# simone7monaco/NO-NODE-comparison

Measured on AMD Instinct MI355X. Metric: N-body trajectories/s (B×T, N=20 rollout) + pos-MSE vs ref, 1/2/4/8 MI355X, higher is better.
Workload: dtype fp32 (fp16x3 split-MFMA, fp32 accumulate, f32 guard); 1 GPU; C2: EGNO forward (4 layers, hidden 64, 2 modes), charged N=20, T=10, B=512 per GPU; batch_per_gpu=512, global_batch=512, n_balls=20, layer_workgroups=256, edges=fixed, parallelism=batch-sharded replicas x1 (no collective)

## Files before the change

### no-node-comparison_amd/csrc/nonode.hip

```cpp
#include "nonode_common.h"

namespace nonode_tu {
thread_local std::string g_err;
}

namespace {

struct ProfState {
  std::mutex mu;
  bool on = false;
  int cap = 0, n = 0;
  hipEvent_t* ev = nullptr;
  int* kind = nullptr;
} g_prof;

constexpr int PROF_SIM_CHARGED = 4, PROF_SIM_GRAVITY = 5, PROF_EDGE_BWD0 = 6, PROF_EDGE_BWD1 = 7;

struct ProfScope {
  int slot = -1;
  hipStream_t s;
  ProfScope(int kind, hipStream_t stream) : s(stream) {
    if (!g_prof.on) return;
    std::lock_guard<std::mutex> lk(g_prof.mu);
    if (g_prof.n >= g_prof.cap) return;
// ... 147 lines not shown
#else
#define STAMP_DECL
#define STAMP(i) do {} while (0)
#define STAMP_FLUSH
#endif

enum { EGNO = 0, SEGNO = 1 };

struct LayerArgs {
  const float* __restrict__ h; const float* __restrict__ x; const float* __restrict__ v;
  const float* __restrict__ ef; const float* __restrict__ blob;
  float* h_out; float* x_out; float* v_out;
  float* pp_h[2]; float* pp_x[2]; float* pp_v[2];
  int steps;
  int fuse, keep;
  float* m_out; float* f_out;
  float* sv_h; float* sv_x; float* sv_v;
  long long sv_n;
  int n_total, n_graphs, N, ne, ef_mod, recurrent;
  int cg, cpg, n_units, ct, s_rows;
  float inv_deg, dt, cw;
  int use_perm;
  unsigned short chunk_of[256];
};

size_t layer_lds_floats(int ct, int s_rows, int keep = 0) {
  return 8192 + EDGE_STAGE_FLOATS + (size_t)ct * 16 * ROWP * 3 + (size_t)s_rows * (ROWP + 4) +
         (size_t)ct * 16 * 4 * 2 + (keep ? (size_t)ct * 16 * (ROWP + 4) : 0);
}

#ifndef NONODE_NODE_PAIR
#define NONODE_NODE_PAIR 1
#endif
template <int VARIANT, int KF, int NW, bool OPT, bool SAVE = false>
__device__ __forceinline__ void egnn_layer_body(const LayerArgs& p, int (*s_cut)[NW + 1]) {
  constexpr bool PAIR = NW == 4;
  constexpr bool TRIPLE = PAIR && VARIANT == EGNO;
  [[maybe_unused]] constexpr bool stamp_here = VARIANT == EGNO && NW == 4 && !OPT;
  constexpr bool rnorm = OPT && VARIANT == EGNO;
  constexpr bool ctanh = OPT && VARIANT == SEGNO;
  extern __shared__ __attribute__((aligned(16))) float smem[];
  const int tid = threadIdx.x, lane = tid & 63, wave = tid >> 6, e = lane & 15, g = lane >> 4;
  const int N = p.N, Nm1 = N - 1;
  float* sW = smem;
  float* sV = sW + 8192;
  float* sP = sV + EDGE_STAGE_FLOATS;
  float* sQ = sP + p.ct * 16 * ROWP;
  float* sX = sQ + p.s_rows * ROWP;
  float* sM = sX + p.s_rows * 4;
  float* sF = sM + 2 * p.ct * 16 * ROWP;
  const int slotM = p.ct * 16 * ROWP, slotF = p.ct * 16 * 4;
  float* sH = sF + 2 * slotF;
  float* sVl = sH + p.ct * 16 * ROWP;
  const bool fused = VARIANT == SEGNO && p.fuse != 0, keep = fused && p.keep != 0;

  for (int i = tid; i < 2048; i += NW * 64) reinterpret_cast<f4*>(sW)[i] = reinterpret_cast<const f4*>(p.blob + OFF_H16)[i];
  if (tid < EDGE_STAGE_FLOATS / 4)
    reinterpret_cast<f4*>(sV)[tid] = reinterpret_cast<const f4*>(p.blob + OFF_FEAT)[tid];
  const float bc2 = p.blob[OFF_SCAL + 0];
  const float bv2 = p.blob[OFF_SCAL + 1];
  const unsigned us_w2 = h16_us(p.blob + OFF_SCAL, HS_W2), us_wc1 = h16_us(p.blob + OFF_SCAL, HS_WC1);
  const float* vFEAT_ = sV;
  const float* vB2_ = sV + 512 + V_B2 * 64;
  const float* vBC1_ = sV + 512 + V_BC1 * 64;
  const float* vWC2_ = sV + 512 + V_WC2 * 64;

  const int G = gridDim.x;
  const int cb = p.use_perm ? (int)p.chunk_of[blockIdx.x] : (int)blockIdx.x;
  const int ch0 = (int)(((long long)cb * p.n_units) / G) * p.cpg;
  const int ch1 = (int)(((long long)(cb + 1) * p.n_units) / G) * p.cpg;
  __syncthreads();
  for (int i = tid; i < 2 * p.ct * 16 * ROWP; i += NW * 64) sM[i] = 0.f;
  for (int i = tid; i < 2 * p.ct * 16 * 4; i += NW * 64) sF[i] = 0.f;
  auto chunk_at = [&](int ci, int& rbase, int& nend, int& s0, int& S) __attribute__((always_inline)) {
    if (p.cpg == 1) {
      const int g_lo = ci * p.cg, g_hi = min(g_lo + p.cg, p.n_graphs);
      rbase = g_lo * N; nend = g_hi * N; s0 = rbase; S = nend - rbase;
    } else {
      const int gi = ci / p.cpg, part = ci - gi * p.cpg;
      s0 = gi * N; S = N;
      rbase = s0 + part * 16 * p.ct; nend = min(rbase + 16 * p.ct, s0 + N);
    }
  };
  auto proj_jobs = [&](int rbase, int nend, int S) __attribute__((always_inline)) {
    const int ctc = (nend - rbase + 15) >> 4;
    return p.cpg == 1 ? ctc : ctc + ((S + 15) >> 4);
  };
  auto proj_tile = [&](const f4 (&hin)[4], const float* blob, int local, bool valid) __attribute__((always_inline)) {
    f4 ap[4], aq[4];
    load_vp(ap, blob + OFF_VEC + V_B1 * 64, g);
#pragma unroll
    for (int mt = 0; mt < 4; ++mt) aq[mt] = f4{0.f, 0.f, 0.f, 0.f};
    if (__builtin_expect(__any(amax_ecl(hin) > H16_LIMIT), 0)) {
      mfma_dense<4>(ap, blob + OFF_WA, hin, lane);
      mfma_dense<4>(aq, blob + OFF_WB, hin, lane);
    } else {
      h8 xh[2], xl[2];
      h16_split(hin, xh, xl);
      mfma_h16(ap, reinterpret_cast<const h8*>(blob + OFF_H16N + H_WA * 4096), xh, xl, lane, h16_us(blob + OFF_SCAL, HS_N + H_WA));
      mfma_h16(aq, reinterpret_cast<const h8*>(blob + OFF_H16N + H_WB * 4096), xh, xl, lane, h16_us(blob + OFF_SCAL, HS_N + H_WB));
    }
    float sa = 0.f;
#pragma unroll
    for (int mt = 0; mt < 4; ++mt)
#pragma unroll
      for (int q = 0; q < 4; ++q) sa += fabsf(ap[mt][q]) + fabsf(aq[mt][q]);
    sa = group_sum(sa);
    if (valid) {
      store_ecl(sP + local * ROWP, ap, g);
      store_ecl(sQ + local * ROWP, aq, g);
      if (g == 0) sX[local * 4 + 3] = __builtin_isfinite(sa) ? 1.f : 0.f;
    }
  };
  auto proj_job = [&](const float* __restrict__ hI, const float* blob, int rbase, int nend, int s0, int S,
                      int job) __attribute__((always_inline)) {
    int joff = 0;
    asm volatile("" : "+s"(joff));
    blob += joff;
    if (p.cpg == 1) {
      const int local = job * 16 + e;
      const bool valid = rbase + local < nend;
      f4 hin[4];
      load_ecl(hin, hI + (size_t)(valid ? rbase + local : nend - 1) * HID, g);
      if (keep && valid) store_ecl(sH + local * ROWP, hin, g);
      proj_tile(hin, blob, local, valid);
      return;
    }
    const int ctc = (nend - rbase + 15) >> 4;
    const bool isP = job < ctc;
    const int local = (isP ? job : job - ctc) * 16 + e;
    int node = isP ? rbase + local : s0 + local;
    const bool valid = isP ? (node < nend) : (local < S);
    node = valid ? node : (isP ? nend - 1 : s0);
    f4 hin[4];
    load_ecl(hin, hI + (size_t)node * HID, g);
    f4 acc[4];
    if (isP) {
      load_vp(acc, blob + OFF_VEC + V_B1 * 64, g);
    } else {
#pragma unroll
      for (int mt = 0; mt < 4; ++mt) acc[mt] = f4{0.f, 0.f, 0.f, 0.f};
    }
    mm64(acc, reinterpret_cast<const h8*>(blob + OFF_H16N + (isP ? H_WA : H_WB) * 4096),
         blob + (isP ? OFF_WA : OFF_WB), hin, lane, h16_us(blob + OFF_SCAL, HS_N + (isP ? H_WA : H_WB)));
    float sa = 0.f;
#pragma unroll
    for (int mt = 0; mt < 4; ++mt)
#pragma unroll
// ... 23 lines not shown
    load_vp(ap0, blob + OFF_VEC + V_B1 * 64, g);
    load_vp(ap1, blob + OFF_VEC + V_B1 * 64, g);
#pragma unroll
    for (int mt = 0; mt < 4; ++mt) aq0[mt] = aq1[mt] = f4{0.f, 0.f, 0.f, 0.f};
    h8 ah[2], al[2], bh[2], bl[2];
    h16_split(h0, ah, al);
    h16_split(h1, bh, bl);
    mfma_h16x2(ap0, ap1, reinterpret_cast<const h8*>(blob + OFF_H16N + H_WA * 4096), ah, al, bh, bl, lane,
               h16_us(blob + OFF_SCAL, HS_N + H_WA));
    mfma_h16x2(aq0, aq1, reinterpret_cast<const h8*>(blob + OFF_H16N + H_WB * 4096), ah, al, bh, bl, lane,
               h16_us(blob + OFF_SCAL, HS_N + H_WB));
    float sa0 = 0.f, sa1 = 0.f;
#pragma unroll
    for (int mt = 0; mt < 4; ++mt)
#pragma unroll
      for (int q = 0; q < 4; ++q) {
        sa0 += fabsf(ap0[mt][q]) + fabsf(aq0[mt][q]);
        sa1 += fabsf(ap1[mt][q]) + fabsf(aq1[mt][q]);
      }
    sa0 = group_sum(sa0);
    sa1 = group_sum(sa1);
    if (v0) {
      store_ecl(sP + l0 * ROWP, ap0, g);
      store_ecl(sQ + l0 * ROWP, aq0, g);
      if (g == 0) sX[l0 * 4 + 3] = __builtin_isfinite(sa0) ? 1.f : 0.f;
    }
    if (v1) {
      store_ecl(sP + l1 * ROWP, ap1, g);
      store_ecl(sQ + l1 * ROWP, aq1, g);
      if (g == 0) sX[l1 * 4 + 3] = __builtin_isfinite(sa1) ? 1.f : 0.f;
    }
  };
  auto load_sx = [&](const float* __restrict__ xI, const float* __restrict__ vI, int s0, int S) __attribute__((always_inline)) {
    for (int i = tid; i < S * 3; i += NW * 64) {
      const int s = i / 3, d = i - 3 * s;
      sX[s * 4 + d] = xI[(size_t)(s0 + s) * 3 + d];
      if (keep) sVl[s * 4 + d] = vI[(size_t)(s0 + s) * 3 + d];
    }
  };
  STAMP_DECL
  int* cut = s_cut[wave];
  int cut_ctc = -1, cut_vl = -1;
  #pragma unroll 1
  for (int step = 0; step < p.steps; ++step) {
  constexpr bool save = VARIANT == SEGNO && SAVE;
  const bool last = step == p.steps - 1;
  const float* __restrict__ hI = step == 0 ? p.h : (save ? p.sv_h + step * p.sv_n * HID : p.pp_h[(step - 1) & 1]);
  const float* __restrict__ xI = step == 0 ? p.x : (save ? p.sv_x + step * p.sv_n * 3 : p.pp_x[(step - 1) & 1]);
  const float* __restrict__ vI = step == 0 ? p.v : (save ? p.sv_v + step * p.sv_n * 3 : p.pp_v[(step - 1) & 1]);
  float* hO = save ? p.sv_h + (step + 1) * p.sv_n * HID : (last ? p.h_out : p.pp_h[step & 1]);
  float* xO = save ? p.sv_x + (step + 1) * p.sv_n * 3 : (last ? p.x_out : p.pp_x[step & 1]);
  float* vO = save ? p.sv_v + (step + 1) * p.sv_n * 3 : (last ? p.v_out : p.pp_v[step & 1]);
  float* mO = p.m_out ? p.m_out + (save ? step * p.sv_n * HID : 0) : nullptr;
  if (!fused || step == 0) {
    int rbase, nend, s0, S;
    chunk_at(ch0, rbase, nend, s0, S);
    load_sx(xI, vI, s0, S);
    const int J = proj_jobs(rbase, nend, S);
    if (NONODE_NODE_PAIR && NW == 4 && VARIANT == EGNO && p.cpg == 1) {
      #pragma unroll 1
      for (int job = 2 * wave; job < J; job += 2 * NW) {
        if (job + 1 < J) proj_job2(hI, p.blob, rbase, nend, job);
        else proj_job(hI, p.blob, rbase, nend, s0, S, job);
      }
    } else {
      #pragma unroll 1
      for (int job = wave; job < J; job += NW) proj_job(hI, p.blob, rbase, nend, s0, S, job);
    }
    STAMP(6);
    __syncthreads();
    STAMP(7);
  }
  #pragma unroll 1
  for (int ci = ch0; ci < ch1; ++ci) {
    int boff = 0;
    asm volatile("" : "+s"(boff));
    const float* blob = p.blob + boff;
    int rbase, nend, s0, S;
    chunk_at(ci, rbase, nend, s0, S);
    const int ctc = (nend - rbase + 15) >> 4;

    {
      const int Vl = (nend - rbase) - 16 * (ctc - 1);
      const int Pk = (Vl <= 4 && Nm1 >= 8) ? 4 : ((Vl <= 8 && Nm1 >= 4) ? 2 : 1);
      const int Kp = Nm1 / Pk;
      const int Ul = Pk == 1 ? Nm1 : Kp + (Nm1 - Pk * Kp);
      const int U = (ctc - 1) * Nm1 + Ul;
      if (ctc != cut_ctc || Vl != cut_vl) {
        cut_ctc = ctc;
        cut_vl = Vl;
        if constexpr (PAIR) {
          unit_split<NW>(ctc, Nm1, Ul, Pk == 1 ? Nm1 : Kp, cut);
        } else {
          const int NWB = min(NW, 3 * ctc);
          for (int i = 0; i <= NW; ++i) cut[i] = i < NWB ? (i * U) / NWB : U;
        }
      }
      const int u1 = cut[wave + 1];
      int u = cut[wave];
      f4 rB2[4], rBC1[4], rWC2[4];
      if (PAIR) {
        load_vp(rB2, vB2_, g);
        load_vp(rBC1, vBC1_, g);
        load_vp(rWC2, vWC2_, g);
      }
      #pragma unroll 1
      while (u < u1) {
        const int tau = min(u / Nm1, ctc - 1);
        const int k_lo = u - tau * Nm1 + 1;
        const int k_hi = min(tau == ctc - 1 ? Ul : Nm1, k_lo + (u1 - u) - 1);
        u += k_hi - k_lo + 1;
        const int P = tau == ctc - 1 ? Pk : 1;
        const int Kq = P == 1 ? Nm1 : Kp;
        const int hp = P == 1 ? 0 : (P == 2 ? e >> 3 : e >> 2);
        const int ee = P == 1 ? e : (P == 2 ? e & 7 : e & 3);
        const int kof = hp * Kq;
        const int kreg = (P - 1) * Kq;
        const int rl = 16 * tau + ee;
        auto lane_k = [&](int k) __attribute__((always_inline)) { return k <= Kq ? k + kof : k + kreg; };
        auto lane_on = [&](int k) __attribute__((always_inline)) { return k <= Kq || hp == 0; };
        const int r = rbase + rl;
        const bool rvalid = r < nend;
        const int rc = rvalid ? r : nend - 1;
        const int gr = rc / N;
        const int n = rc - gr * N;
        const int sb = gr * N - s0;
        const size_t ebase = ((size_t)(gr % p.ef_mod) * N + n) * Nm1;
        int voff = 0;
        asm volatile("" : "+v"(voff));
        const float* vFEAT = vFEAT_ + voff;
        const float* Prow = sP + rl * ROWP;
        const float xr0 = sX[(sb + n) * 4 + 0], xr1 = sX[(sb + n) * 4 + 1], xr2 = sX[(sb + n) * 4 + 2];
        const float xr3 = sX[(sb + n) * 4 + 3];
        f4 msum[4];
#pragma unroll
        for (int mt = 0; mt < 4; ++mt) msum[mt] = f4{0.f, 0.f, 0.f, 0.f};
        float fs0 = 0.f, fs1 = 0.f, fs2 = 0.f;

        const float* ef_seg = p.ef + ebase * p.ne;
        int ef_lane[KF];
#pragma unroll
        for (int kf = 0; kf < KF; ++kf) ef_lane[kf] = n * p.ne + min(max(4 * kf + g - 1, 0), p.ne - 1);
        const int ne_wrap = N * p.ne;
        auto fetch_ef = [&](int k, float (&ev)[KF]) __attribute__((always_inline)) {
          const int sub = (n + k >= N) ? ne_wrap : p.ne;
          const int kne = k * p.ne;
#pragma unroll
          for (int kf = 0; kf < KF; ++kf)
            ev[kf] = ef_seg[ef_lane[kf] + kne - sub];
        };
        auto head = [&](int k, const float (&ev)[KF], f4 (&a)[4], float& r0, float& r1, float& r2)
            __attribute__((always_inline)) {
          int j = n + k;
          j = (j >= N) ? j - N : j;
          const int sl = sb + j;
          const float* xs = sX + sl * 4;
          r0 = xr0 - xs[0]; r1 = xr1 - xs[1]; r2 = xr2 - xs[2];
          float d2 = fmaf(r0, r0, fmaf(r1, r1, r2 * r2));
          if constexpr (rnorm) d2 = radial_norm(d2);
          f4 q4[4];
// ... 242 lines not shown
#pragma unroll
              for (int mo = 0; mo < 4; ++mo) a[mo] = mfma(wf[mo], bv, a[mo]);
            }
          };
          auto coord1 = [&](f4 (&c1)[4], const float* wc2, float r0, float r1, float r2, float& f0, float& f1,
                            float& f2, float& c) __attribute__((always_inline)) {
            silu_ecl(c1);
            c = dot_vp(c1, wc2, g) + bc2;
            float ct = c;
            if constexpr (ctanh) ct = tanhf(c);
            f0 = r0 * ct; f1 = r1 * ct; f2 = r2 * ct;
            if (VARIANT == SEGNO) {
              f0 = fminf(fmaxf(f0, -100.f), 100.f);
              f1 = fminf(fmaxf(f1, -100.f), 100.f);
              f2 = fminf(fmaxf(f2, -100.f), 100.f);
            }
          };
          auto unit1 = [&](int k, int k_end, float (&e0)[KF], auto masked) __attribute__((always_inline)) {
            float en[KF];
            fetch_ef(lane_k(min(k + 1, k_end)), en);
            int loff = 0;
            asm volatile("" : "+v"(loff));
            const h8* w2l = w2h + loff;
            const h8* wc1l = wc1h + loff;
            f4 a[4], m[4];
            float r0, r1, r2, f0, f1, f2, c;
            bool ok;
            head1(lane_k(k), e0, a, r0, r1, r2, ok);
            silu_ecl(a);
            load_vp(m, vB2_ + loff, g);
            {
              h8 ah[2], al[2];
              h16_split(a, ah, al);
              mfma_h16(m, w2l, ah, al, lane, us_w2);
            }
            silu_ecl(m);
            load_vp(a, vBC1_ + loff, g);
            {
              h8 mh[2], ml[2];
              h16_split(m, mh, ml);
              mfma_h16(a, wc1l, mh, ml, lane, us_wc1);
            }
            coord1(a, vWC2_ + loff, r0, r1, r2, f0, f1, f2, c);
            if (__builtin_expect(__any(ok && !__builtin_isfinite(c)), 0)) {
              int kg = k;
              asm volatile("" : "+v"(kg));
              head1(lane_k(kg), e0, a, r0, r1, r2, ok);
              silu_ecl(a);
              load_vp(m, vB2_, g);
              mm64_scaled(m, w2h, a, lane, us_w2);
              silu_ecl(m);
              load_vp(a, vBC1_, g);
              mm64_scaled(a, wc1h, m, lane, us_wc1);
              coord1(a, vWC2_, r0, r1, r2, f0, f1, f2, c);
            }
            if constexpr (decltype(masked)::value) {
              const bool on = lane_on(k);
#pragma unroll
              for (int mt = 0; mt < 4; ++mt)
#pragma unroll
                for (int q = 0; q < 4; ++q) msum[mt][q] = on ? msum[mt][q] + m[mt][q] : msum[mt][q];
              fs0 = on ? fs0 + f0 : fs0; fs1 = on ? fs1 + f1 : fs1; fs2 = on ? fs2 + f2 : fs2;
            } else {
#pragma unroll
              for (int mt = 0; mt < 4; ++mt) msum[mt] += m[mt];
              fs0 += f0; fs1 += f1; fs2 += f2;
            }
#pragma unroll
            for (int kf = 0; kf < KF; ++kf) e0[kf] = en[kf];
          };
          float e0[KF];
          fetch_ef(lane_k(min(k, k_hi)), e0);
          const int ko_hi = min(k_hi, Kq);
#pragma unroll 1
          for (; k <= ko_hi; ++k) unit1(k, ko_hi, e0, std::false_type{});
          if (k <= k_hi) fetch_ef(lane_k(k), e0);
#pragma unroll 1
          for (; k <= k_hi; ++k) unit1(k, k_hi, e0, std::true_type{});
        }
        float e0[KF];
        fetch_ef(lane_k(min(k, k_hi)), e0);
        STAMP(8);
#pragma unroll 1
        for (; k <= k_hi; ++k) {
          float en[KF];
          fetch_ef(lane_k(min(k + 1, k_hi)), en);
          const bool on = lane_on(k);
          int loff = 0;
          asm volatile("" : "+v"(loff));
          const h8* w2l = w2h + loff;
          const h8* wc1l = wc1h + loff;
          const float* vB2l = vB2_ + loff;
          const float* vBC1l = vBC1_ + loff;
          f4 a[4], m[4];
          float r0, r1, r2;
          head(lane_k(k), e0, a, r0, r1, r2);
#pragma unroll
          for (int kf = 0; kf < KF; ++kf) e0[kf] = en[kf];
          STAMP(0);
          silu_ecl(a);
          if (PAIR) {
#pragma unroll
            for (int mt = 0; mt < 4; ++mt) m[mt] = rB2[mt];
          } else {
            load_vp(m, vB2l, g);
          }
          if (__builtin_expect(__any(amax_ecl(a) > H16_LIMIT), 0)) {
            mm64_scaled(m, w2l, a, lane, us_w2);
          } else {
            h8 ah[2], al[2];
            h16_split(a, ah, al);
            mfma_h16(m, w2l, ah, al, lane, us_w2);
          }
          STAMP(1);
          silu_ecl(m);
#pragma unroll
          for (int mt = 0; mt < 4; ++mt)
#pragma unroll
            for (int q = 0; q < 4; ++q) msum[mt][q] = on ? msum[mt][q] + m[mt][q] : msum[mt][q];
          if (PAIR) {
#pragma unroll
            for (int mt = 0; mt < 4; ++mt) a[mt] = rBC1[mt];
          } else {
            load_vp(a, vBC1l, g);
          }
          if (__builtin_expect(__any(amax_ecl(m) > H16_LIMIT), 0)) {
            mm64_scaled(a, wc1l, m, lane, us_wc1);
          } else {
            h8 mh[2], ml[2];
            h16_split(m, mh, ml);
            mfma_h16(a, wc1l, mh, ml, lane, us_wc1);
          }
          STAMP(2);
          tail(a, r0, r1, r2, on);
          STAMP(3);
        }
        if (P > 1) {
#pragma unroll
          for (int mt = 0; mt < 4; ++mt)
#pragma unroll
            for (int q = 0; q < 4; ++q) msum[mt][q] = group_fold(msum[mt][q], P);
          fs0 = group_fold(fs0, P); fs1 = group_fold(fs1, P); fs2 = group_fold(fs2, P);
        }
        const int t0 = tau * Nm1, t1 = t0 + (tau == ctc - 1 ? Ul : Nm1);
        bool solo = true;
#pragma unroll
        for (int w = 0; w < NW; ++w)
          if (w != wave && ((w ^ wave) & 1) == 0 && cut[w] < cut[w + 1] && cut[w] < t1 && cut[w + 1] > t0)
            solo = false;
        if (rvalid && hp == 0) {
          const int slot = wave & 1;
          float* mrow = sM + slot * slotM + rl * ROWP;
          float* frow = sF + slot * slotF + rl * 4;
          if (solo) {
            store_ecl(mrow, msum, g);
            if (g == 0) *reinterpret_cast<f4*>(frow) = f4{fs0, fs1, fs2, 0.f};
          } else {
#pragma unroll
            for (int mt = 0; mt < 4; ++mt)
#pragma unroll
              for (int q = 0; q < 4; ++q) atomicAdd(mrow + 16 * mt + 4 * g + q, msum[mt][q]);
            if (g == 0) {
              atomicAdd(frow + 0, fs0);
              atomicAdd(frow + 1, fs1);
              atomicAdd(frow + 2, fs2);
            }
          }
        }
        STAMP(9);
      }
    }
    STAMP(10);
    __syncthreads();
    STAMP(11);

    {
      const bool has_next = ci + 1 < ch1;
      int nrb = 0, nne = 0, ns0 = 0, nS = 0;
      if (has_next) {
        chunk_at(ci + 1, nrb, nne, ns0, nS);
        load_sx(xI, vI, ns0, nS);
      }
#ifndef NONODE_C_COST
#define NONODE_C_COST 4
#endif
#ifndef NONODE_A_COST
#define NONODE_A_COST 2
#endif
#ifndef NONODE_CP_COST
#define NONODE_CP_COST 8
#endif
#ifndef NONODE_AP_COST
#define NONODE_AP_COST 4
#endif
      constexpr bool PAIR = NONODE_NODE_PAIR != 0 && NW == 4 && VARIANT == EGNO;
      const int PJ = has_next ? proj_jobs(nrb, nne, nS) : 0;
      const bool ppair = PAIR && p.cpg == 1;
      const int NJN = PAIR ? (ctc + 1) >> 1 : ctc;
      const int J = NJN + (ppair ? (PJ + 1) >> 1 : PJ);
      constexpr int C_COST = NONODE_C_COST;
      const int A_COST = p.cpg == 1 ? NONODE_A_COST : 1;
      int ld[NW];
#pragma unroll
      for (int i = 0; i < NW; ++i) ld[i] = 0;
      auto node_job = [&](auto U_, const float* bj, int tau0) __attribute__((always_inline)) {
        constexpr int U = decltype(U_)::value;
        int rl[U], r[U], lc[U];
        bool rvalid[U];
        f4 hr[U][4], Mr[U][4];
        float F0[U], F1[U], F2[U], x0[U], x1[U], x2[U], v0[U], v1[U], v2[U];
#pragma unroll
        for (int u = 0; u < U; ++u) {
          rl[u] = 16 * (tau0 + u) + e;
          r[u] = rbase + rl[u];
          rvalid[u] = r[u] < nend;
          const int rc = rvalid[u] ? r[u] : nend - 1;
          lc[u] = rc - rbase;
          f4 Mb[4];
          if (keep) load_ecl(hr[u], sH + lc[u] * ROWP, g);
          else load_ecl(hr[u], hI + (size_t)rc * HID, g);
          load_ecl(Mr[u], sM + rl[u] * ROWP, g);
          load_ecl(Mb, sM + slotM + rl[u] * ROWP, g);
#pragma unroll
          for (int mt = 0; mt < 4; ++mt) Mr[u][mt] += Mb[mt];
          const float* fa = sF + rl[u] * 4;
          const float* fb = sF + slotF + rl[u] * 4;
          F0[u] = fa[0] + fb[0]; F1[u] = fa[1] + fb[1]; F2[u] = fa[2] + fb[2];
          {
            const f4 z4[4] = {};
            store_ecl(sM + rl[u] * ROWP, z4, g);
            store_ecl(sM + slotM + rl[u] * ROWP, z4, g);
            if (g == 0) {
              *reinterpret_cast<f4*>(sF + rl[u] * 4) = z4[0];
              *reinterpret_cast<f4*>(sF + slotF + rl[u] * 4) = z4[0];
            }
          }
          if (fused) { x0[u] = sX[lc[u] * 4 + 0]; x1[u] = sX[lc[u] * 4 + 1]; x2[u] = sX[lc[u] * 4 + 2]; }
          else { const size_t gr3 = (size_t)rc * 3; x0[u] = xI[gr3 + 0]; x1[u] = xI[gr3 + 1]; x2[u] = xI[gr3 + 2]; }
// ... 122 lines not shown
      #pragma unroll 1
      for (int j = 0; j < J; ++j) {
        int w = 0, lw = ld[0];
#pragma unroll
        for (int i = 1; i < NW; ++i)
          if (ld[i] < lw) { lw = ld[i]; w = i; }
        const bool nodej = j < NJN;
        const int first = nodej ? (PAIR ? 2 * j : j) : (ppair ? 2 * (j - NJN) : j - NJN);
        const bool two = nodej ? (PAIR && first + 1 < ctc) : (ppair && first + 1 < PJ);
        const int c = nodej ? (two ? NONODE_CP_COST : C_COST) : (two ? NONODE_AP_COST : A_COST);
#pragma unroll
        for (int i = 0; i < NW; ++i) ld[i] += i == w ? c : 0;
        if (w != wave) continue;
        int joff = 0;
        asm volatile("" : "+s"(joff));
        const float* bj = blob + joff;
        if (!nodej) {
          if (two) proj_job2(hI, bj, nrb, nne, first);
          else proj_job(hI, bj, nrb, nne, ns0, nS, first);
          continue;
        }
        if (two) node_job(std::integral_constant<int, 2>{}, bj, first);
        else node_job(std::integral_constant<int, 1>{}, bj, first);
      }
    }
    STAMP(12);
    __syncthreads();
    STAMP(13);
  }
  }
  STAMP_FLUSH
}

template <int VARIANT, int KF, int NW>
__global__ __launch_bounds__(NW * 64) void egnn_layer_kernel(LayerArgs p) {
  __shared__ int s_cut[NW][NW + 1];
  if constexpr (VARIANT == SEGNO) {
    if (p.sv_h) {
      if (p.blob[OFF_SCAL + SC_TANH] != 0.f) egnn_layer_body<VARIANT, KF, NW, true, true>(p, s_cut);
      else egnn_layer_body<VARIANT, KF, NW, false, true>(p, s_cut);
      return;
    }
  }
  if (p.blob[OFF_SCAL + (VARIANT == SEGNO ? SC_TANH : SC_NORM)] != 0.f)
    egnn_layer_body<VARIANT, KF, NW, true>(p, s_cut);
  else
    egnn_layer_body<VARIANT, KF, NW, false>(p, s_cut);
}

struct TconvArgs {
  int BN, T, M, Mfull;
  const float* h; const float* x; const float* v; const float* lm;
  const float* wp;
  const float* wx;
  float* h_out; float* x_out; float* v_out;
  const float* hin; int din; const float* emb_w; int emb_ld; const float* etab; int Bt;
  int frames;
  int xcd;
  int xw;
  unsigned long long* mask_out;
  float tw_cos[MMAX * TMAX], tw_sin[MMAX * TMAX];
};

constexpr int tconv_mats(int M) { return 1 + 3 * (M - 1); }
size_t tconv_blob_floats(int modes) { return (size_t)tconv_mats(modes) * 8192 + 128; }
__device__ __forceinline__ size_t tconv_h16_off(int M) { return (size_t)tconv_mats(M) * 4096; }
__device__ __forceinline__ size_t tconv_scal_off(int M) { return (size_t)tconv_mats(M) * 8192; }

struct TconvPackBatch { const float* w[PACK_MAX]; float* out[PACK_MAX]; };
__global__ void tconv_pack_kernel(TconvPackBatch tb, int Mfull, int M, int T) {
  const float* w = tb.w[blockIdx.y];
  float* out = tb.out[blockIdx.y];
  const int d = blockIdx.x * blockDim.x + threadIdx.x;
  const int nmat = 1 + 3 * (M - 1);
  if (d >= nmat * 4096) return;
  const int mat = d >> 12, r = d & 4095;
  const int q = r & 3, l = (r >> 2) & 63, rest = r >> 8, mt = rest & 3, mo = rest >> 2;
  const int o = 16 * mo + (l & 15), i = 16 * mt + 4 * (l >> 4) + q;
  int m, c;
  float sgn = 1.f;
// ... 360 lines not shown
  const int idx = blockIdx.x * blockDim.x + threadIdx.x;
  if (idx >= BN * 64) return;
  const int o = idx & 63, c = idx >> 6;
  auto hin_part = [&](size_t r) {
    float b = 0.f;
    for (int k = 0; k < din; ++k) b = fmaf(emb_w[o * emb_ld + k], hin[r * din + k], b);
    return b;
  };
  const float base = frames ? 0.f : hin_part((size_t)c);
  const float* et = etab + (size_t)(c % Bt) * T * 64 + o;
  float e[TMAX];
#pragma unroll
  for (int t = 0; t < TMAX; ++t) e[t] = t < T ? et[t * 64] : 0.f;
#pragma unroll
  for (int t = 0; t < TMAX; ++t) {
    if (t >= T) break;
    const size_t row = (size_t)t * BN + c;
    const size_t src = frames ? row : (size_t)c;
    h0[row * 64 + o] = e[t] + (frames ? hin_part(row) : base);
    if (o < 3) { xr[row * 3 + o] = x[src * 3 + o]; vr[row * 3 + o] = v[src * 3 + o]; }
    if (hin_out && o < din && (frames || t == 0)) hin_out[src * din + o] = hin[src * din + o];
  }
}

constexpr int LAYER_DYN_LDS_MAX = 159 * 1024;
int getenv_int(const char* name) {
  const char* v = getenv(name);
  return v ? atoi(v) : 0;
}
bool xcd_on() {
  static const int on = getenv("NONODE_XCD") ? atoi(getenv("NONODE_XCD")) : 1;
  return on != 0;
}
template <int VARIANT, int NW>
void launch_cfg(int kf, int G, size_t lds, hipStream_t stream, const LayerArgs& a) {
  static std::once_flag once;
  std::call_once(once, [] {
    hipFuncSetAttribute((const void*)egnn_layer_kernel<VARIANT, 1, NW>, hipFuncAttributeMaxDynamicSharedMemorySize, LAYER_DYN_LDS_MAX);
    hipFuncSetAttribute((const void*)egnn_layer_kernel<VARIANT, 2, NW>, hipFuncAttributeMaxDynamicSharedMemorySize, LAYER_DYN_LDS_MAX);
  });
  if (kf == 1) hipLaunchKernelGGL((egnn_layer_kernel<VARIANT, 1, NW>), dim3(G), dim3(NW * 64), lds, stream, a);
  else hipLaunchKernelGGL((egnn_layer_kernel<VARIANT, 2, NW>), dim3(G), dim3(NW * 64), lds, stream, a);
}
#ifndef NONODE_LAYER_WAVES
#define NONODE_LAYER_WAVES 0
#endif
template <int VARIANT>
int launch_layer(int n_graphs, int N, int ne, int ef_mod, const float* h, const float* x,
                 const float* v, const float* ef, const float* blob, float dt, float cw, int recurrent,
                 float* h_out, float* x_out, float* v_out, hipStream_t stream, int steps = 1,
                 float* const* pp = nullptr, float* m_out = nullptr, float* f_out = nullptr,
                 int xcd_cols = 0, float* const* sv = nullptr) {
  const int n_total = n_graphs * N;
  const int cus = num_cus();
  constexpr size_t LDS_MAX = LAYER_DYN_LDS_MAX;
  const int cap = n_graphs / cus > 1 ? n_graphs / cus : 1;
  int cg = 0, cpg = 1, ct = 0;
  double best = -1.0;
  const bool crit = steps == 1 && !m_out && !sv && n_graphs < 16 * cus && !getenv_int("NONODE_FILL_CG");
  const int force_cg = getenv_int("NONODE_CG");
  if (crit) best = -1e300;
  for (int c = 1; c <= (crit || force_cg ? 8 * 16 : cap); ++c) {
    if (force_cg) {
      const int tiles = (c * N + 15) / 16;
      if (tiles > 8 || layer_lds_floats(tiles, c * N) * 4 > LDS_MAX) break;
      cg = c; ct = tiles;
      if (c == force_cg) break;
      continue;
    }
    const int tiles = (c * N + 15) / 16;
    if (tiles > 8 || layer_lds_floats(tiles, c * N) * 4 > LDS_MAX) break;
    if (crit) {
      const long long chunks = (n_graphs + c - 1) / c;
      const long long rounds = (chunks + cus - 1) / cus;
      const double cost = -(double)rounds * (tiles + 0.5);
      if (cost > best + 1e-12) { best = cost; cg = c; ct = tiles; }
      continue;
    }
    const double fill = (double)(c * N) / (16.0 * tiles);
// ... 19 lines not shown
  a.n_total = n_total; a.n_graphs = n_graphs; a.N = N; a.ne = ne; a.ef_mod = ef_mod;
  a.cg = cg; a.cpg = cpg; a.n_units = n_units; a.ct = ct; a.s_rows = s_rows;
  if (steps < 1 || (steps > 1 && !pp && !sv)) return fail(NONODE_EINVAL, "layer: steps=%d", steps);
  a.steps = steps;
  a.fuse = fuse && !getenv_int("NONODE_NO_FUSE");
  a.keep = a.fuse && keep;
  a.m_out = m_out; a.f_out = f_out;
  a.sv_h = sv ? sv[0] : nullptr; a.sv_x = sv ? sv[1] : nullptr; a.sv_v = sv ? sv[2] : nullptr;
  a.sv_n = n_total;
  for (int i = 0; i < 2; ++i) {
    a.pp_h[i] = pp ? pp[i] : nullptr;
    a.pp_x[i] = pp ? pp[2 + i] : nullptr;
    a.pp_v[i] = pp ? pp[4 + i] : nullptr;
  }
  a.recurrent = recurrent; a.inv_deg = 1.0f / (float)(N - 1); a.dt = dt; a.cw = cw;
  a.use_perm = 0;
  if (xcd_cols > 0 && G % 8 == 0 && G <= 256 && xcd_on()) {
    int slot_fill[8] = {0};
    int left[256], nleft = 0;
    for (int k = 0; k < G; ++k) a.chunk_of[k] = 0xffff;
    for (int c = 0; c < G; ++c) {
      const long long row0 = (((long long)c * n_units) / G) * cg * N;
      const int x = (int)((row0 % xcd_cols) * 8 / xcd_cols);
      if (slot_fill[x] < G / 8) a.chunk_of[x + 8 * slot_fill[x]++] = (unsigned short)c;
      else left[nleft++] = c;
    }
    for (int k = 0, i = 0; k < G; ++k)
      if (a.chunk_of[k] == 0xffff) a.chunk_of[k] = (unsigned short)left[i++];
    a.use_perm = 1;
  }
  ProfScope prof(VARIANT, stream);
  if (ne == 0) { a.ef = blob; a.ne = 1; a.ef_mod = 1; }
  const int kf = a.ne <= 3 ? 1 : 2;
  const int nw = NONODE_LAYER_WAVES ? NONODE_LAYER_WAVES : (N < 64 ? 4 : 8);
  if (nw == 8) launch_cfg<VARIANT, 8>(kf, G, lds, stream, a);
  else launch_cfg<VARIANT, 4>(kf, G, lds, stream, a);
  return check_launch("egnn_layer_kernel");
}

void cos_sin_pi(int num, int den, double& c, double& s) {
  num %= 2 * den;
  if ((2 * num) % den == 0) {
    const int q = (2 * num) / den;
    const double cq[4] = {1.0, 0.0, -1.0, 0.0}, sq[4] = {0.0, 1.0, 0.0, -1.0};
    c = cq[q]; s = sq[q];
    return;
  }
  const double ang = 3.14159265358979323846 * (double)num / (double)den;
  c = cos(ang); s = sin(ang);
}
int launch_tconv(bool first, const TconvArgs& a_in, hipStream_t stream) {
  TconvArgs a = a_in;
  for (int m = 0; m < MMAX; ++m)
    for (int t = 0; t < TMAX; ++t) {
      double c = 0.0, sn = 0.0;
      if (m < a.M && t < a.T) cos_sin_pi(2 * m * t, a.T, c, sn);
      a.tw_cos[m * TMAX + t] = (float)c;
      a.tw_sin[m * TMAX + t] = (float)sn;
    }
  const int ntiles = (a.BN + 15) / 16;
  a.xcd = xcd_on() && ntiles >= 64;
  a.xw = ntiles < num_cus() && !getenv_int("NONODE_TC_NOXW");
  const int grid = a.xcd ? 8 * ((ntiles + 7) / 8) : ntiles;
  ProfScope prof(first ? 3 : 2, stream);
  auto go = [&](auto kt, auto kf) {
    const int threads = a.xw ? TC_THREADS : 256;
    if (first) hipLaunchKernelGGL(kt, dim3(grid), dim3(threads), 0, stream, a);
    else hipLaunchKernelGGL(kf, dim3(grid), dim3(threads), 0, stream, a);
// ... 371 lines not shown
```

### no-node-comparison_amd/csrc/nonode_common.h

```cpp
#pragma once
#include <hip/hip_runtime.h>

#include <cmath>
#include <cstdarg>
#include <cstdio>
#include <cstdlib>
#include <cstring>
#include <mutex>
#include <string>
#include <type_traits>
#include <vector>

#include "nonode.h"

namespace nonode_tu {
extern thread_local std::string g_err;
}

namespace {

using nonode_tu::g_err;

typedef float f4 __attribute__((ext_vector_type(4)));
typedef _Float16 h8 __attribute__((ext_vector_type(8)));
// ... 195 lines not shown

__device__ __forceinline__ void mm64(f4 (&acc)[4], const h8* wh, const float* wf, const f4 (&x)[4], int lane,
                                     unsigned us) {
  if (__builtin_expect(__any(amax_ecl(x) > H16_LIMIT), 0)) {
    mfma_dense<4>(acc, wf, x, lane);
  } else {
    h8 xh[2], xl[2];
    h16_split(x, xh, xl);
    mfma_h16(acc, wh, xh, xl, lane, us);
  }
}

struct H16Frags {
  h8 hi[2][4], lo[2][4];
};
__device__ __forceinline__ void load_h16frags(H16Frags& f, const h8* wf, int lane) {
#pragma unroll
  for (int s = 0; s < 2; ++s)
#pragma unroll
    for (int mo = 0; mo < 4; ++mo) {
      f.hi[s][mo] = wf[((s * 4 + mo) * 2 + 0) * 64 + lane];
      f.lo[s][mo] = wf[((s * 4 + mo) * 2 + 1) * 64 + lane];
    }
}
__device__ __forceinline__ void pin_agpr(H16Frags& f) {
#pragma unroll
  for (int s = 0; s < 2; ++s)
#pragma unroll
    for (int mo = 0; mo < 4; ++mo) {
      asm volatile("" : "+a"(f.hi[s][mo]));
      asm volatile("" : "+a"(f.lo[s][mo]));
    }
}
__device__ __forceinline__ void mfma_h16r2(f4 (&acc0)[4], f4 (&acc1)[4], const H16Frags& f, const h8 (&x0h)[2],
                                           const h8 (&x0l)[2], const h8 (&x1h)[2], const h8 (&x1l)[2], unsigned us) {
#pragma unroll
  for (int s = 0; s < 2; ++s) {
    const h8 x0s = h8_scale(x0h[s], us), x1s = h8_scale(x1h[s], us);
#pragma unroll
    for (int mo = 0; mo < 4; ++mo) { acc0[mo] = mfma16(f.hi[s][mo], x0h[s], acc0[mo]); acc1[mo] = mfma16(f.hi[s][mo], x1h[s], acc1[mo]); }
#pragma unroll
    for (int mo = 0; mo < 4; ++mo) { acc0[mo] = mfma16(f.lo[s][mo], x0s, acc0[mo]); acc1[mo] = mfma16(f.lo[s][mo], x1s, acc1[mo]); }
#pragma unroll
    for (int mo = 0; mo < 4; ++mo) { acc0[mo] = mfma16(f.hi[s][mo], x0l[s], acc0[mo]); acc1[mo] = mfma16(f.hi[s][mo], x1l[s], acc1[mo]); }
  }
}

__device__ __forceinline__ void mfma_h16r3(f4 (&acc0)[4], f4 (&acc1)[4], f4 (&acc2)[4], const H16Frags& f,
                                           const h8 (&x0h)[2], const h8 (&x0l)[2], const h8 (&x1h)[2],
                                           const h8 (&x1l)[2], const h8 (&x2h)[2], const h8 (&x2l)[2], unsigned us) {
#pragma unroll
  for (int s = 0; s < 2; ++s) {
    const h8 x0s = h8_scale(x0h[s], us), x1s = h8_scale(x1h[s], us), x2s = h8_scale(x2h[s], us);
#pragma unroll
    for (int mo = 0; mo < 4; ++mo) {
      acc0[mo] = mfma16(f.hi[s][mo], x0h[s], acc0[mo]);
      acc1[mo] = mfma16(f.hi[s][mo], x1h[s], acc1[mo]);
      acc2[mo] = mfma16(f.hi[s][mo], x2h[s], acc2[mo]);
    }
#pragma unroll
    for (int mo = 0; mo < 4; ++mo) {
      acc0[mo] = mfma16(f.lo[s][mo], x0s, acc0[mo]);
      acc1[mo] = mfma16(f.lo[s][mo], x1s, acc1[mo]);
      acc2[mo] = mfma16(f.lo[s][mo], x2s, acc2[mo]);
    }
#pragma unroll
// ... 144 lines not shown
    if (unit_fill<NW>(mid, ctc, Nm1, Ul, Ql, cut)) hi = mid;
    else lo = mid + 1;
  }
  unit_fill<NW>(lo, ctc, Nm1, Ul, Ql, cut);
}
__device__ __forceinline__ float group_max(float v) {
  const auto a = __builtin_amdgcn_permlane32_swap(__float_as_uint(v), __float_as_uint(v), false, false);
  v = fmaxf(__uint_as_float(a[0]), __uint_as_float(a[1]));
  const auto b = __builtin_amdgcn_permlane16_swap(__float_as_uint(v), __float_as_uint(v), false, false);
  return fmaxf(__uint_as_float(b[0]), __uint_as_float(b[1]));
}
__device__ __forceinline__ void mm64_scaled(f4 (&acc)[4], const H16Frags& f, const f4 (&x)[4], unsigned us) {
  const float cmax = group_max(amax_ecl(x));
  const int s = max(__builtin_amdgcn_frexp_expf(cmax) - 13, 0);
  const float dn = __uint_as_float((unsigned)(127 - s) << 23), up = __uint_as_float((unsigned)(127 + min(s, 127)) << 23);
  f4 xs[4], t[4];
#pragma unroll
  for (int mt = 0; mt < 4; ++mt) { xs[mt] = x[mt] * dn; t[mt] = f4{0.f, 0.f, 0.f, 0.f}; }
  h8 xh[2], xl[2];
  h16_split(xs, xh, xl);
#pragma unroll
  for (int k = 0; k < 2; ++k) {
    const h8 xs2 = h8_scale(xh[k], us);
#pragma unroll
    for (int mo = 0; mo < 4; ++mo) t[mo] = mfma16(f.hi[k][mo], xh[k], t[mo]);
#pragma unroll
    for (int mo = 0; mo < 4; ++mo) t[mo] = mfma16(f.lo[k][mo], xs2, t[mo]);
#pragma unroll
    for (int mo = 0; mo < 4; ++mo) t[mo] = mfma16(f.hi[k][mo], xl[k], t[mo]);
  }
#pragma unroll
  for (int mt = 0; mt < 4; ++mt) acc[mt] += t[mt] * up;
}
__device__ __forceinline__ void mm64_scaled(f4 (&acc)[4], const h8* wh, const f4 (&x)[4], int lane, unsigned us) {
  const float cmax = group_max(amax_ecl(x));
  const int s = max(__builtin_amdgcn_frexp_expf(cmax) - 13, 0);
  const float dn = __uint_as_float((unsigned)(127 - s) << 23), up = __uint_as_float((unsigned)(127 + min(s, 127)) << 23);
  f4 xs[4], t[4];
#pragma unroll
  for (int mt = 0; mt < 4; ++mt) { xs[mt] = x[mt] * dn; t[mt] = f4{0.f, 0.f, 0.f, 0.f}; }
  h8 xh[2], xl[2];
  h16_split(xs, xh, xl);
  mfma_h16(t, wh, xh, xl, lane, us);
#pragma unroll
  for (int mt = 0; mt < 4; ++mt) acc[mt] += t[mt] * up;
}

__device__ __forceinline__ unsigned h16_us(const float* scal, int idx) {
  return __float_as_uint(scal[SC_H16S + idx]);
}

}
```

Baseline: 581,400 trajectories/s.

## Keep EGNO edge-MLP weight fragments register-resident in an 8-wave layer variant

```diff
diff --git a/no-node-comparison_amd/csrc/nonode.hip b/no-node-comparison_amd/csrc/nonode.hip
--- a/no-node-comparison_amd/csrc/nonode.hip
+++ b/no-node-comparison_amd/csrc/nonode.hip
@@ -203,15 +203,25 @@
 #ifndef NONODE_NODE_PAIR
 #define NONODE_NODE_PAIR 1
 #endif
-template <int VARIANT, int KF, int NW, bool OPT, bool SAVE = false>
+#define LANE_IDS_FRESH                                                 \
+  int lane_f_ = lane0_;                                                \
+  if constexpr (RES) asm volatile("" : "+v"(lane_f_));                 \
+  [[maybe_unused]] const int lane = lane_f_, e = RES ? lane_f_ & 15 : e0_, g = RES ? lane_f_ >> 4 : g0_;
+#ifndef NONODE_RES_MASK
+#define NONODE_RES_MASK 7
+#endif
+template <int VARIANT, int KF, int NW, bool OPT, bool SAVE = false, bool RES = false>
 __device__ __forceinline__ void egnn_layer_body(const LayerArgs& p, int (*s_cut)[NW + 1]) {
   constexpr bool PAIR = NW == 4;
+  constexpr bool R2H = RES && (NONODE_RES_MASK & 1), R2L = RES && (NONODE_RES_MASK & 2);
+  constexpr bool RCH = RES && (NONODE_RES_MASK & 4), RCL = RES && (NONODE_RES_MASK & 8);
   constexpr bool TRIPLE = PAIR && VARIANT == EGNO;
   [[maybe_unused]] constexpr bool stamp_here = VARIANT == EGNO && NW == 4 && !OPT;
   constexpr bool rnorm = OPT && VARIANT == EGNO;
   constexpr bool ctanh = OPT && VARIANT == SEGNO;
   extern __shared__ __attribute__((aligned(16))) float smem[];
   const int tid = threadIdx.x, lane = tid & 63, wave = tid >> 6, e = lane & 15, g = lane >> 4;
+  const int lane0_ = lane, e0_ = e, g0_ = g, tid0_ = tid;
   const int N = p.N, Nm1 = N - 1;
   float* sW = smem;
   float* sV = sW + 8192;
@@ -258,6 +268,7 @@
     return p.cpg == 1 ? ctc : ctc + ((S + 15) >> 4);
   };
   auto proj_tile = [&](const f4 (&hin)[4], const float* blob, int local, bool valid) __attribute__((always_inline)) {
+    LANE_IDS_FRESH
     f4 ap[4], aq[4];
     load_vp(ap, blob + OFF_VEC + V_B1 * 64, g);
 #pragma unroll
@@ -285,6 +296,7 @@
   };
   auto proj_job = [&](const float* __restrict__ hI, const float* blob, int rbase, int nend, int s0, int S,
                       int job) __attribute__((always_inline)) {
+    LANE_IDS_FRESH
     int joff = 0;
     asm volatile("" : "+s"(joff));
     blob += joff;
@@ -374,6 +386,9 @@
     }
   };
   auto load_sx = [&](const float* __restrict__ xI, const float* __restrict__ vI, int s0, int S) __attribute__((always_inline)) {
+    int tid_f_ = tid0_;
+    if constexpr (RES) asm volatile("" : "+v"(tid_f_));
+    const int tid = tid_f_;
     for (int i = tid; i < S * 3; i += NW * 64) {
       const int s = i / 3, d = i - 3 * s;
       sX[s * 4 + d] = xI[(size_t)(s0 + s) * 3 + d];
@@ -434,20 +449,36 @@
         if constexpr (PAIR) {
           unit_split<NW>(ctc, Nm1, Ul, Pk == 1 ? Nm1 : Kp, cut);
         } else {
-          const int NWB = min(NW, 3 * ctc);
+          int NWB = min(NW, 3 * ctc);
+          if constexpr (RES) {
+            const int r = (Nm1 - 2) / 3 + 1;
+            NWB = max(1, min(NW, U / r));
+          }
           for (int i = 0; i <= NW; ++i) cut[i] = i < NWB ? (i * U) / NWB : U;
         }
       }
-      const int u1 = cut[wave + 1];
+      int u1 = cut[wave + 1];
       int u = cut[wave];
+      if constexpr (RES) {
+        u1 = __builtin_amdgcn_readfirstlane(u1);
+        u = __builtin_amdgcn_readfirstlane(u);
+      }
       f4 rB2[4], rBC1[4], rWC2[4];
       if (PAIR) {
         load_vp(rB2, vB2_, g);
         load_vp(rBC1, vBC1_, g);
         load_vp(rWC2, vWC2_, g);
       }
+      H16Frags rw2, rwc1;
+      if constexpr (RES) {
+        int foff = 0;
+        asm volatile("" : "+v"(foff));
+        load_h16part<R2H, R2L>(rw2, reinterpret_cast<const h8*>(sW) + foff, lane);
+        load_h16part<RCH, RCL>(rwc1, reinterpret_cast<const h8*>(sW + 4096) + foff, lane);
+      }
       #pragma unroll 1
       while (u < u1) {
+        LANE_IDS_FRESH
         const int tau = min(u / Nm1, ctc - 1);
         const int k_lo = u - tau * Nm1 + 1;
         const int k_hi = min(tau == ctc - 1 ? Ul : Nm1, k_lo + (u1 - u) - 1);
@@ -464,10 +495,12 @@
         const int r = rbase + rl;
         const bool rvalid = r < nend;
         const int rc = rvalid ? r : nend - 1;
-        const int gr = rc / N;
+        int Nd = N, efd = p.ef_mod;
+        if constexpr (RES) asm volatile("" : "+s"(Nd), "+s"(efd));
+        const int gr = rc / Nd;
         const int n = rc - gr * N;
         const int sb = gr * N - s0;
-        const size_t ebase = ((size_t)(gr % p.ef_mod) * N + n) * Nm1;
+        const size_t ebase = ((size_t)(gr % efd) * N + n) * Nm1;
         int voff = 0;
         asm volatile("" : "+v"(voff));
         const float* vFEAT = vFEAT_ + voff;
@@ -776,14 +809,16 @@
             {
               h8 ah[2], al[2];
               h16_split(a, ah, al);
-              mfma_h16(m, w2l, ah, al, lane, us_w2);
+              if constexpr (RES) mfma_h16m<R2H, R2L>(m, rw2, w2l, ah, al, lane, us_w2);
+              else mfma_h16(m, w2l, ah, al, lane, us_w2);
             }
             silu_ecl(m);
             load_vp(a, vBC1_ + loff, g);
             {
               h8 mh[2], ml[2];
               h16_split(m, mh, ml);
-              mfma_h16(a, wc1l, mh, ml, lane, us_wc1);
+              if constexpr (RES) mfma_h16m<RCH, RCL>(a, rwc1, wc1l, mh, ml, lane, us_wc1);
+              else mfma_h16(a, wc1l, mh, ml, lane, us_wc1);
             }
             coord1(a, vWC2_ + loff, r0, r1, r2, f0, f1, f2, c);
             if (__builtin_expect(__any(ok && !__builtin_isfinite(c)), 0)) {
@@ -792,10 +827,12 @@
               head1(lane_k(kg), e0, a, r0, r1, r2, ok);
               silu_ecl(a);
               load_vp(m, vB2_, g);
-              mm64_scaled(m, w2h, a, lane, us_w2);
+              if constexpr (RES) mm64_scaled_m<R2H, R2L>(m, rw2, w2h, a, lane, us_w2);
+              else mm64_scaled(m, w2h, a, lane, us_w2);
               silu_ecl(m);
               load_vp(a, vBC1_, g);
-              mm64_scaled(a, wc1h, m, lane, us_wc1);
+              if constexpr (RES) mm64_scaled_m<RCH, RCL>(a, rwc1, wc1h, m, lane, us_wc1);
+              else mm64_scaled(a, wc1h, m, lane, us_wc1);
               coord1(a, vWC2_, r0, r1, r2, f0, f1, f2, c);
             }
             if constexpr (decltype(masked)::value) {
@@ -823,10 +860,10 @@
           for (; k <= k_hi; ++k) unit1(k, k_hi, e0, std::true_type{});
         }
         float e0[KF];
-        fetch_ef(lane_k(min(k, k_hi)), e0);
+        if constexpr (!RES) fetch_ef(lane_k(min(k, k_hi)), e0);
         STAMP(8);
 #pragma unroll 1
-        for (; k <= k_hi; ++k) {
+        for (; !RES && k <= k_hi; ++k) {
           float en[KF];
           fetch_ef(lane_k(min(k + 1, k_hi)), en);
           const bool on = lane_on(k);
@@ -879,6 +916,8 @@
           tail(a, r0, r1, r2, on);
           STAMP(3);
         }
+        {
+        LANE_IDS_FRESH
         if (P > 1) {
 #pragma unroll
           for (int mt = 0; mt < 4; ++mt)
@@ -910,6 +949,7 @@
               atomicAdd(frow + 2, fs2);
             }
           }
+        }
         }
         STAMP(9);
       }
@@ -948,6 +988,7 @@
 #pragma unroll
       for (int i = 0; i < NW; ++i) ld[i] = 0;
       auto node_job = [&](auto U_, const float* bj, int tau0) __attribute__((always_inline)) {
+        LANE_IDS_FRESH
         constexpr int U = decltype(U_)::value;
         int rl[U], r[U], lc[U];
         bool rvalid[U];
@@ -1136,8 +1177,9 @@
   STAMP_FLUSH
 }
 
-template <int VARIANT, int KF, int NW>
+template <int VARIANT, int KF, int NW, bool RES = false>
 __global__ __launch_bounds__(NW * 64) void egnn_layer_kernel(LayerArgs p) {
+  static_assert(!RES || (NW == 8 && VARIANT == EGNO), "register-resident fragments: the 8-wave EGNO layer");
   __shared__ int s_cut[NW][NW + 1];
   if constexpr (VARIANT == SEGNO) {
     if (p.sv_h) {
@@ -1147,9 +1189,9 @@
     }
   }
   if (p.blob[OFF_SCAL + (VARIANT == SEGNO ? SC_TANH : SC_NORM)] != 0.f)
-    egnn_layer_body<VARIANT, KF, NW, true>(p, s_cut);
+    egnn_layer_body<VARIANT, KF, NW, true, false, RES>(p, s_cut);
   else
-    egnn_layer_body<VARIANT, KF, NW, false>(p, s_cut);
+    egnn_layer_body<VARIANT, KF, NW, false, false, RES>(p, s_cut);
 }
 
 struct TconvArgs {
@@ -1576,19 +1618,28 @@
   static const int on = getenv("NONODE_XCD") ? atoi(getenv("NONODE_XCD")) : 1;
   return on != 0;
 }
-template <int VARIANT, int NW>
+template <int VARIANT, int NW, bool RES = false>
 void launch_cfg(int kf, int G, size_t lds, hipStream_t stream, const LayerArgs& a) {
   static std::once_flag once;
   std::call_once(once, [] {
-    hipFuncSetAttribute((const void*)egnn_layer_kernel<VARIANT, 1, NW>, hipFuncAttributeMaxDynamicSharedMemorySize, LAYER_DYN_LDS_MAX);
-    hipFuncSetAttribute((const void*)egnn_layer_kernel<VARIANT, 2, NW>, hipFuncAttributeMaxDynamicSharedMemorySize, LAYER_DYN_LDS_MAX);
+    hipFuncSetAttribute((const void*)egnn_layer_kernel<VARIANT, 1, NW, RES>, hipFuncAttributeMaxDynamicSharedMemorySize, LAYER_DYN_LDS_MAX);
+    hipFuncSetAttribute((const void*)egnn_layer_kernel<VARIANT, 2, NW, RES>, hipFuncAttributeMaxDynamicSharedMemorySize, LAYER_DYN_LDS_MAX);
   });
-  if (kf == 1) hipLaunchKernelGGL((egnn_layer_kernel<VARIANT, 1, NW>), dim3(G), dim3(NW * 64), lds, stream, a);
-  else hipLaunchKernelGGL((egnn_layer_kernel<VARIANT, 2, NW>), dim3(G), dim3(NW * 64), lds, stream, a);
-}
-#ifndef NONODE_LAYER_WAVES
-#define NONODE_LAYER_WAVES 0
+  if (kf == 1) hipLaunchKernelGGL((egnn_layer_kernel<VARIANT, 1, NW, RES>), dim3(G), dim3(NW * 64), lds, stream, a);
+  else hipLaunchKernelGGL((egnn_layer_kernel<VARIANT, 2, NW, RES>), dim3(G), dim3(NW * 64), lds, stream, a);
+}
+#ifndef NONODE_LAYER_RES_DEFAULT
+#define NONODE_LAYER_RES_DEFAULT 1
 #endif
+constexpr bool LAYER_RES_DEFAULT = NONODE_LAYER_RES_DEFAULT != 0;
+int layer_waves_forced() {
+  static const int w = getenv_int("NONODE_LAYER_WAVES");
+  return w == 4 || w == 8 ? w : 0;
+}
+bool layer_nores() {
+  static const int v = getenv_int("NONODE_LAYER_NORES");
+  return v != 0;
+}
 template <int VARIANT>
 int launch_layer(int n_graphs, int N, int ne, int ef_mod, const float* h, const float* x,
                  const float* v, const float* ef, const float* blob, float dt, float cw, int recurrent,
@@ -1674,8 +1725,16 @@
   ProfScope prof(VARIANT, stream);
   if (ne == 0) { a.ef = blob; a.ne = 1; a.ef_mod = 1; }
   const int kf = a.ne <= 3 ? 1 : 2;
-  const int nw = NONODE_LAYER_WAVES ? NONODE_LAYER_WAVES : (N < 64 ? 4 : 8);
-  if (nw == 8) launch_cfg<VARIANT, 8>(kf, G, lds, stream, a);
+  const int forced = layer_waves_forced();
+  const bool res_ok = VARIANT == EGNO && N < 64;
+  const int nw = forced ? forced : (N >= 64 || (res_ok && LAYER_RES_DEFAULT) ? 8 : 4);
+  bool res = false;
+  if constexpr (VARIANT == EGNO) res = nw == 8 && res_ok && !layer_nores();
+  if constexpr (VARIANT == EGNO) {
+    if (res) launch_cfg<VARIANT, 8, true>(kf, G, lds, stream, a);
+  }
+  if (res) {}
+  else if (nw == 8) launch_cfg<VARIANT, 8>(kf, G, lds, stream, a);
   else launch_cfg<VARIANT, 4>(kf, G, lds, stream, a);
   return check_launch("egnn_layer_kernel");
 }
diff --git a/no-node-comparison_amd/csrc/nonode_common.h b/no-node-comparison_amd/csrc/nonode_common.h
--- a/no-node-comparison_amd/csrc/nonode_common.h
+++ b/no-node-comparison_amd/csrc/nonode_common.h
@@ -251,6 +251,38 @@
       asm volatile("" : "+a"(f.lo[s][mo]));
     }
 }
+template <bool RH, bool RL>
+__device__ __forceinline__ void load_h16part(H16Frags& f, const h8* wf, int lane) {
+#pragma unroll
+  for (int s = 0; s < 2; ++s)
+#pragma unroll
+    for (int mo = 0; mo < 4; ++mo) {
+      if constexpr (RH) { f.hi[s][mo] = wf[((s * 4 + mo) * 2 + 0) * 64 + lane]; asm volatile("" : "+v"(f.hi[s][mo])); }
+      if constexpr (RL) { f.lo[s][mo] = wf[((s * 4 + mo) * 2 + 1) * 64 + lane]; asm volatile("" : "+v"(f.lo[s][mo])); }
+    }
+}
+template <bool RH, bool RL>
+__device__ __forceinline__ void mfma_h16m(f4 (&acc)[4], const H16Frags& f, const h8* wf, const h8 (&xh)[2],
+                                          const h8 (&xl)[2], int lane, unsigned us) {
+#pragma unroll
+  for (int s = 0; s < 2; ++s) {
+    h8 ah[4], al[4];
+#pragma unroll
+    for (int mo = 0; mo < 4; ++mo) {
+      if constexpr (RH) ah[mo] = f.hi[s][mo];
+      else ah[mo] = wf[((s * 4 + mo) * 2 + 0) * 64 + lane];
+      if constexpr (RL) al[mo] = f.lo[s][mo];
+      else al[mo] = wf[((s * 4 + mo) * 2 + 1) * 64 + lane];
+    }
+    const h8 xs = h8_scale(xh[s], us);
+#pragma unroll
+    for (int mo = 0; mo < 4; ++mo) acc[mo] = mfma16(ah[mo], xh[s], acc[mo]);
+#pragma unroll
+    for (int mo = 0; mo < 4; ++mo) acc[mo] = mfma16(al[mo], xs, acc[mo]);
+#pragma unroll
+    for (int mo = 0; mo < 4; ++mo) acc[mo] = mfma16(ah[mo], xl[s], acc[mo]);
+  }
+}
 __device__ __forceinline__ void mfma_h16r2(f4 (&acc0)[4], f4 (&acc1)[4], const H16Frags& f, const h8 (&x0h)[2],
                                            const h8 (&x0l)[2], const h8 (&x1h)[2], const h8 (&x1l)[2], unsigned us) {
 #pragma unroll
@@ -461,6 +493,21 @@
 #pragma unroll
   for (int mt = 0; mt < 4; ++mt) acc[mt] += t[mt] * up;
 }
+template <bool RH, bool RL>
+__device__ __forceinline__ void mm64_scaled_m(f4 (&acc)[4], const H16Frags& f, const h8* wh, const f4 (&x)[4], int lane,
+                                              unsigned us) {
+  const float cmax = group_max(amax_ecl(x));
+  const int s = max(__builtin_amdgcn_frexp_expf(cmax) - 13, 0);
+  const float dn = __uint_as_float((unsigned)(127 - s) << 23), up = __uint_as_float((unsigned)(127 + min(s, 127)) << 23);
+  f4 xs[4], t[4];
+#pragma unroll
+  for (int mt = 0; mt < 4; ++mt) { xs[mt] = x[mt] * dn; t[mt] = f4{0.f, 0.f, 0.f, 0.f}; }
+  h8 xh[2], xl[2];
+  h16_split(xs, xh, xl);
+  mfma_h16m<RH, RL>(t, f, wh, xh, xl, lane, us);
+#pragma unroll
+  for (int mt = 0; mt < 4; ++mt) acc[mt] += t[mt] * up;
+}
 __device__ __forceinline__ void mm64_scaled(f4 (&acc)[4], const h8* wh, const f4 (&x)[4], int lane, unsigned us) {
   const float cmax = group_max(amax_ecl(x));
   const int s = max(__builtin_amdgcn_frexp_expf(cmax) - 13, 0);
```

New measurement: 545,500 trajectories/s. -6.2%, worse.
